# fusioninfer/fusioninfer

Hardware: NVIDIA H100
Metric: routing decisions/sec (4K-tok prompts x 1024 endpoints); achieved HBM GB/s (higher is better)
Workload: dtype u64

## Files before the change

fusioninfer_b200/csrc/engine.cu:

```cuda
#include <cuda_runtime.h>
#include <unistd.h>
#include <dlfcn.h>

#include <algorithm>
#include <atomic>
#include <chrono>
#include <cmath>
#include <condition_variable>
#include <cstdio>
#include <cstdlib>
#include <cstring>
#include <functional>
#include <memory>
#include <mutex>
#include <string>
#include <thread>
#include <unordered_set>
#include <vector>

#include <sched.h>

#include "../../include/fi_epp.h"
#include "cuda_owned.h"
#include "kernels.cuh"
// ... 149 lines not shown

  fi_epp_config cfg;
  std::mutex mu;
  std::string err;
  int sm_count = 132;
  uint32_t MP = 0;
  uint32_t W = 0;
  uint32_t P = 0;
  bool fast_hash = false;

  static constexpr int kMaxFeedSlices = 16;
  Event ev_copy[kMaxFeedSlices];
  uint32_t feed_slices = 8;
  DevPtr<uint64_t> d_chain2;
  DevPtr<uint32_t> d_nblocks2;
  Event ev_in, ev_a[2], ev_b[2];
  Event ev_pick;
  Event ev_plain;
  uint64_t pipe_seq = 0;
  static constexpr int kTicketRing = 8;
  Event ev_ticket[kTicketRing];
  uint64_t tickets = 0;
  uint64_t slot_ticket[2] = {~0ull, ~0ull};
  uint32_t slot_R[2] = {0, 0};
  Event ev_slot_read[2];
  Event ev_index, ev_user, ev_done, ev_ctr;

  DevPtr<uint8_t> d_prompts;
  DevPtr<uint64_t> d_offsets;
  DevPtr<uint64_t> d_h0;
  DevPtr<uint64_t> d_chain;
  DevPtr<uint32_t> d_nblocks;
  DevPtr<fi_pick> d_picks;
  Staging<fi_pick> ranked;
  Staging<uint32_t> subsets;
  Staging<uint16_t> counts;
  std::unique_ptr<ShardState> shard;
  PeerXchg px{};
  bool split_hash = false;
  uint32_t chain_rows = 0;
  DevPtr<unsigned long long> d_probed;
  DevPtr<uint32_t> d_work;
  PinnedPtr<fi_pick> h_picks;
  PinnedPtr<uint64_t> h_offsets;
  PinnedPtr<uint64_t> h_h0;
  PinnedPtr<uint32_t> h_nblocks;

// ... 819 lines not shown
    }
    LaunchScope ls(h, h->s_index.get(), K_INDEX);
    FI_CUDA(launch_index_clear_counted(h->ix.v, h->d_ctr.get(), h->dlru->clears.get(), r_total[k], h->dlru->ctr.get() + 2, lo, EL, h->rank, glog,
                                       h->s_index.get()));
  }
  return update_end(h, Readback::kIndexAndLru);
}

bool early_exit_hashing(const fi_epp* h, bool chains_wanted) {
  return h->world == 1 && h->fast_hash && !chains_wanted && h->cfg.lru_capacity == 0;
}

unsigned long long* hashed_counter(fi_epp* h) { return h->profiling ? h->d_probed.get() + 6 : nullptr; }

int run_hash(fi_epp* h, const uint8_t* d_prompts, const uint64_t* d_offsets, const uint64_t* d_h0, uint32_t r0,
             uint32_t R, cudaStream_t s, const IndexView* early) {
  uint64_t* chain = h->d_chain.get() + (size_t)r0 * h->MP;
  uint32_t* nb = h->d_nblocks.get() + r0;
  LaunchScope ls(h, s, K_HASH);
  if (h->fast_hash) {
    FI_CUDA(launch_hash_chain(d_prompts, d_offsets + r0, d_h0 + r0, R, h->cfg.block_bytes, h->cfg.max_blocks, h->MP,
                              chain, nb, h->sm_count, s, early, hashed_counter(h)));
  } else {
    FI_CUDA(launch_hash_generic(d_prompts, d_offsets + r0, d_h0 + r0, R, h->cfg.block_bytes, h->cfg.max_blocks, h->MP,
                                chain, nb, s));
  }
  return FI_OK;
}

int nccl_allgather_on(fi_epp* h, ncclComm_t comm, const void* send, void* recv, size_t bytes, cudaStream_t s) {
  int rc = g_nccl.AllGather(send, recv, bytes, ncclInt8, comm, s);
  if (rc != ncclSuccess)
    return fail(h, FI_ERR_COMM, std::string("ncclAllGather: ") + (g_nccl.GetErrorString ? g_nccl.GetErrorString(rc) : "error"));
  return FI_OK;
}
int nccl_allgather(fi_epp* h, const void* send, void* recv, size_t bytes) {
  return nccl_allgather_on(h, h->shard->comm, send, recv, bytes, h->s_main.get());
// ... 226 lines not shown
  const uint32_t S = h->feed_slices;
  if (feed && !sharded && h->fast_hash && S > 1 && R >= 64 * S && feed->offsets[R] >= (8ull << 20)) {
    uint8_t* dp = const_cast<uint8_t*>(c.prompts);
    const uint32_t per = (((R + S - 1) / S) + 31) & ~31u;
    uint32_t used = 0;
    for (uint32_t k = 0; k * per < R; ++k, ++used) {
      const uint32_t r0 = k * per, r1 = std::min(R, r0 + per);
      const uint64_t b0 = feed->offsets[r0], b1 = feed->offsets[r1];
      if (b1 > b0) FI_CUDA(cudaMemcpyAsync(dp + b0, feed->prompts + b0, b1 - b0, cudaMemcpyHostToDevice, h->s_copy.get()));
      FI_CUDA(cudaEventRecord(h->ev_copy[k].get(), h->s_copy.get()));
    }
    h->stats.h2d_bytes += feed->offsets[R];
    for (uint32_t k = 0; k < used; ++k) {
      const uint32_t r0 = k * per, Rk = std::min(per, R - r0);
      FI_CUDA(cudaStreamWaitEvent(h->s_main.get(), h->ev_copy[k].get(), 0));
      rc = run_hash(h, c.prompts, c.offsets, c.h0, r0, Rk, h->s_main.get(), early);
      if (rc != FI_OK) return rc;
      MatchParams ms = mp;
      ms.chain = mp.chain + (size_t)r0 * h->MP;
      ms.nblocks = mp.nblocks + r0;
      ms.offsets = mp.offsets ? mp.offsets + r0 : nullptr;
      ms.adapters = mp.adapters ? mp.adapters + r0 : nullptr;
      ms.subsets = mp.subsets ? mp.subsets + (size_t)r0 * mp.sub_pitch : nullptr;
      ms.h0 = mp.h0 + r0;
      ms.r_base = r0;
      ms.R = Rk;
      ms.out = mp.out ? mp.out + (size_t)r0 * h->P * std::max(c.k, 1u) : nullptr;
      ms.counts = mp.counts ? mp.counts + (size_t)r0 * h->cfg.endpoint_count : nullptr;
      ms.work_counter = h->d_work.get() + k;
      LaunchScope ls(h, h->s_main.get(), K_MATCH);
      FI_CUDA(launch_match_pick(ms, h->sm_count, h->s_main.get()));
    }
    return FI_OK;
  }
  if (feed && feed->offsets[R]) {
    FI_CUDA(cudaMemcpyAsync(const_cast<uint8_t*>(c.prompts), feed->prompts, feed->offsets[R], cudaMemcpyHostToDevice, h->s_main.get()));
    h->stats.h2d_bytes += feed->offsets[R];
  }
  if (!sharded) {
    rc = run_hash(h, c.prompts, c.offsets, c.h0, 0, R, h->s_main.get(), early);
    if (rc != FI_OK) return rc;
    LaunchScope ls(h, h->s_main.get(), K_MATCH);
    FI_CUDA(launch_match_pick(mp, h->sm_count, h->s_main.get()));
    return FI_OK;
  }

  if (h->split_hash && h->fast_hash && R >= 32 * h->world) {
    const uint32_t per = (((R + h->world - 1) / h->world) + 31) & ~31u;
    const uint32_t r0 = std::min(R, h->rank * per), r1 = std::min(R, r0 + per);
    if (r1 > r0) {
      rc = run_hash(h, c.prompts, c.offsets, c.h0, r0, r1 - r0, h->s_main.get(), nullptr);
      if (rc != FI_OK) return rc;
    }
    rc = nccl_allgather(h, h->d_chain.get() + (size_t)h->rank * per * h->MP, h->d_chain.get(), (size_t)per * h->MP * sizeof(uint64_t));
    if (rc != FI_OK) return rc;
// ... 60 lines not shown
  return FI_OK;
}

int issue_ticket(fi_epp* h, uint64_t* t) {
  FI_CUDA(cudaEventRecord(h->ev_ticket[h->tickets % fi_epp::kTicketRing].get(), h->s_main.get()));
  *t = h->tickets++;
  return FI_OK;
}

int submit_pick(fi_epp* h, const PickCall& c, cudaStream_t us, uint64_t* ticket, bool lagged) {
  const uint32_t R = c.R;
  int rc = settle_updates(h, lagged);
  if (rc != FI_OK) return rc;
  if (!h->d_chain2) {
    DevPtr<uint64_t> chain;
    DevPtr<uint32_t> nb;
    FI_CUDA(cuda_alloc(chain, (size_t)h->cfg.max_batch * h->MP));
    FI_CUDA(cuda_alloc(nb, h->cfg.max_batch));
    h->d_chain2 = std::move(chain);
    h->d_nblocks2 = std::move(nb);
  }
  if (!h->profiling && h->trace_call >= 0 && (long)h->stats.pick_calls >= h->trace_call &&
      (long)h->stats.pick_calls < h->trace_call + 3) {
    if ((long)h->stats.pick_calls == h->trace_call) {
      if (!h->ev_trace0) cuda_create(h->ev_trace0, cudaEventDefault);
      FI_CUDA(cudaStreamSynchronize(h->s_main.get()));
      FI_CUDA(cudaStreamSynchronize(h->s_a.get()));
      FI_CUDA(cudaEventRecord(h->ev_trace0.get(), h->s_main.get()));
      FI_CUDA(cudaStreamWaitEvent(h->s_a.get(), h->ev_trace0.get(), 0));
    }
    h->tracing = true;
  } else if (h->tracing && (long)h->stats.pick_calls >= h->trace_call + 3) {
    h->tracing = false;
  }
  const uint32_t slot = (uint32_t)(h->pipe_seq & 1);
  uint64_t* chain = slot ? h->d_chain2.get() : h->d_chain.get();
  uint32_t* nb = slot ? h->d_nblocks2.get() : h->d_nblocks.get();
  FI_CUDA(cudaEventRecord(h->ev_in.get(), us));
  FI_CUDA(cudaStreamWaitEvent(h->s_a.get(), h->ev_in.get(), 0));
  if (h->pipe_seq >= 2) FI_CUDA(cudaStreamWaitEvent(h->s_a.get(), h->ev_b[slot].get(), 0));
  FI_CUDA(cudaStreamWaitEvent(h->s_a.get(), h->ev_plain.get(), 0));
  rc = wait_slot_readers(h, slot, h->s_a.get());
  if (rc != FI_OK) return rc;
  MatchParams mp;
  rc = prepare_match(h, c, chain, nb, mp);
  if (rc != FI_OK) return rc;
  const bool early = early_exit_hashing(h, c.chains_out != nullptr);
  if (early) FI_CUDA(cudaStreamWaitEvent(h->s_a.get(), h->ev_index.get(), 0));
  {
    LaunchScope ls(h, h->s_a.get(), K_HASH);
    FI_CUDA(launch_hash_chain(c.prompts, c.offsets, c.h0, R, h->cfg.block_bytes, h->cfg.max_blocks, h->MP, chain, nb,
                              h->sm_count, h->s_a.get(), early ? &mp.ix : nullptr, hashed_counter(h)));
  }
  FI_CUDA(cudaEventRecord(h->ev_a[slot].get(), h->s_a.get()));
  FI_CUDA(cudaStreamWaitEvent(h->s_main.get(), h->ev_a[slot].get(), 0));
  mp.work_counter = h->d_work.get() + 8 + slot;
  {
    LaunchScope ls(h, h->s_main.get(), K_MATCH);
    FI_CUDA(launch_match_pick(mp, h->sm_count, h->s_main.get()));
  }
  rc = copy_chains_out(h, chain, c.chains_out, R, cudaMemcpyDeviceToDevice, h->s_main.get());
  if (rc != FI_OK) return rc;
  FI_CUDA(cudaEventRecord(h->ev_b[slot].get(), h->s_main.get()));
  FI_CUDA(cudaEventRecord(h->ev_pick.get(), h->s_main.get()));
  rc = issue_ticket(h, ticket);
  if (rc != FI_OK) return rc;
  h->slot_ticket[slot] = *ticket;
// ... 212 lines not shown
  if (const char* e = std::getenv("FI_EPP_FEED_SLICES")) {
    const long v = std::strtol(e, nullptr, 10);
    h->feed_slices = (uint32_t)std::min<long>(std::max<long>(v, 1), fi_epp::kMaxFeedSlices);
  }
  for (Event* e : {&h->ev_index, &h->ev_user, &h->ev_done, &h->ev_ctr}) FI_TRY(cuda_create(*e));
  FI_TRY(cudaEventRecord(h->ev_index.get(), h->s_index.get()));
  const uint64_t R = cfg->max_batch;
  h->chain_rows = (uint32_t)((R + 31) / 32 * 32);
  if (cfg->endpoint_count < cfg->num_endpoints) h->chain_rows += 32 * (FI_MAX_RANKS + 1);
  if (const char* e = std::getenv("FI_EPP_SHARD_HASH")) h->split_hash = std::strcmp(e, "split") == 0;
  FI_TRY(cuda_alloc(h->d_prompts, h->cfg.max_prompt_bytes + 64));
  FI_TRY(cuda_alloc(h->d_offsets, R + 1));
  FI_TRY(cuda_alloc(h->d_h0, R));
  FI_TRY(cuda_alloc(h->d_chain, (size_t)h->chain_rows * h->MP));
  FI_TRY(cuda_alloc(h->d_nblocks, h->chain_rows));
  FI_TRY(cuda_alloc(h->d_picks, R * h->P));
  FI_TRY(cuda_alloc(h->d_probed, 8));
  FI_TRY(cudaMemset(h->d_probed.get(), 0, 8 * sizeof(unsigned long long)));
  FI_TRY(cuda_alloc(h->d_work, 16));
  FI_TRY(cudaMemset(h->d_work.get(), 0, 16 * sizeof(uint32_t)));
  FI_TRY(cuda_alloc(h->h_picks, R * h->P));
  FI_TRY(cuda_alloc(h->h_offsets, R + 1));
  FI_TRY(cuda_alloc(h->h_h0, R));
  FI_TRY(cuda_alloc(h->h_nblocks, R));

  FI_TRY(cuda_alloc(h->d_ctr, 1));
  FI_TRY(cudaMemset(h->d_ctr.get(), 0, sizeof(IndexCounters)));
  FI_TRY(cuda_alloc(h->h_ctr, 1));
  std::memset(h->h_ctr.get(), 0, sizeof(IndexCounters));
  {
// ... 1341 lines not shown
```

fusioninfer_b200/csrc/hash_kernels.cu:

```cuda
#include "kernels.cuh"
#include "xxh64.cuh"
#include "xxh64_sm100.cuh"
#include "index_device.cuh"

namespace fi {

namespace {

__device__ __forceinline__ uint64_t make_evict_first_policy() {
  uint64_t pol;
  asm volatile("createpolicy.fractional.L2::evict_first.b64 %0, 1.0;\n" : "=l"(pol));
  return pol;
}
__device__ __forceinline__ uint4 ld_stream_v4(const uint4* p, uint64_t pol) {
  uint4 v;
  asm volatile("ld.global.nc.L1::evict_first.L2::cache_hint.v4.u32 {%0, %1, %2, %3}, [%4], %5;\n"
               : "=r"(v.x), "=r"(v.y), "=r"(v.z), "=r"(v.w)
               : "l"(p), "l"(pol));
  return v;
}

struct Stripe {
  uint32_t w[8];
};
// ... 55 lines not shown
  const uint32_t sh = (uint32_t)(addr & 7) * 8;
  XAcc2 a = xacc2_init();
  if constexpr (STRIPES == 0) {
#pragma unroll 2
    for (uint32_t s = 0; s < B / 32; ++s) xacc2_stripe_at(a, wp + 4 * (uint64_t)s, sh);
  } else {
#pragma unroll
    for (int s = 0; s < STRIPES; ++s) xacc2_stripe_at(a, wp + 4 * s, sh);
  }
  return xacc2_finish(a, (uint64_t)B + 8);
}

enum : int { kHashFull = 0, kHashFullCounted = 1, kHashEarly = 2 };

__device__ __forceinline__ uint32_t ld_volatile_shared(const uint32_t* p) { return *reinterpret_cast<const volatile uint32_t*>(p); }
__device__ __forceinline__ uint64_t ld_chain_cta(const uint64_t* p) {
  uint64_t v;
  asm volatile("ld.relaxed.cta.global.u64 %0, [%1];\n" : "=l"(v) : "l"(p) : "memory");
  return v;
}

template <int STRIPES, int WALK, int WARPS, int MODE>
__global__ void __launch_bounds__(WARPS * 32, 32 / WARPS) hash_chain_kernel(const uint8_t* __restrict__ prompts,
                                                                   const uint64_t* __restrict__ offsets,
                                                                   const uint64_t* __restrict__ h0, uint32_t R,
                                                                   uint32_t M, uint32_t MP,
                                                                   uint64_t* __restrict__ chain,
                                                                   uint32_t* __restrict__ nblocks,
                                                                   uint32_t block_bytes, const IndexView ix,
                                                                   unsigned long long* hashed) {
  constexpr bool EARLY = MODE == kHashEarly;
  const uint32_t B = STRIPES ? STRIPES * 32 : block_bytes;
  constexpr uint32_t BPL = STRIPES == 4 || STRIPES == 0 ? 1 : 2;
  constexpr uint32_t kFuseReq = 32 * WALK;
  constexpr uint32_t kFuseHashWarps = WARPS - WALK - (EARLY ? 1 : 0);
  constexpr uint32_t kFuseRing = WARPS * kFuseRingBytesPerWarp / (WALK * 4 * 32 * 16);
  constexpr uint32_t kJobs = kFuseReq / (4 * BPL);
  __shared__ __align__(16) ulonglong2 s_ring[kFuseRing][WALK][4][32];
  __shared__ uint64_t s_full[kFuseRing], s_empty[kFuseRing];
  __shared__ const uint8_t* s_base[kFuseReq];
  __shared__ uint32_t s_n[kFuseReq];
  __shared__ uint32_t s_groups;
  __shared__ uint32_t s_stop[EARLY ? kFuseReq : 1], s_walked[EARLY ? WALK : 1], s_hashed;

  const uint32_t tid = threadIdx.x, lane = tid & 31, warp = tid >> 5;
  const uint32_t r_tile = blockIdx.x * kFuseReq;
  if (tid == 0) {
    s_groups = 0;
    for (uint32_t s = 0; s < kFuseRing; ++s) {
      mbar_init(&s_full[s], kJobs * 32);
      mbar_init(&s_empty[s], WALK * 32);
    }
    if constexpr (EARLY)
      for (uint32_t w = 0; w < WALK; ++w) s_walked[w] = 0;
    if constexpr (MODE != kHashFull) s_hashed = 0;
  }
  __syncthreads();
  if (tid < kFuseReq) {
    const uint32_t r = r_tile + tid;
    uint32_t n = 0;
    const uint8_t* base = prompts;
    if (r < R) {
      const uint64_t off = offsets[r];
      const uint64_t nb64 = (offsets[r + 1] - off) / B;
      n = nb64 > M ? M : (uint32_t)nb64;
      base = prompts + off;
      nblocks[r] = n;
    }
    s_n[tid] = n;
    s_base[tid] = base;
    if constexpr (EARLY) s_stop[tid] = 0xFFFFFFFFu;
    if constexpr (MODE == kHashFullCounted)
      if (n) atomicAdd(&s_hashed, n);
    atomicMax(&s_groups, (n + 7) / 8);
  }
  __syncthreads();
  const uint32_t ng = s_groups;
  if constexpr (MODE == kHashFullCounted)
    if (tid == 0 && s_hashed) atomicAdd(hashed, (unsigned long long)s_hashed);

  if constexpr (EARLY) {
    if (warp == WALK) {
      uint32_t done_g[WALK];
      bool live[WALK];
#pragma unroll
      for (int j = 0; j < WALK; ++j) {
        done_g[j] = 0;
        live[j] = r_tile + j * 32 + lane < R && s_n[j * 32 + lane] > 0;
      }
#pragma unroll 1
      for (;;) {
        uint32_t gw[WALK];
        bool any = false, fresh = false;
#pragma unroll
        for (int j = 0; j < WALK; ++j) {
          gw[j] = ld_volatile_shared(&s_walked[j]);
          live[j] = live[j] && done_g[j] * 8 < s_n[j * 32 + lane];
          any = any || live[j];
          fresh = fresh || (live[j] && gw[j] > done_g[j]);
        }
        if (!__any_sync(0xFFFFFFFFu, any)) break;
        if (!__any_sync(0xFFFFFFFFu, fresh)) {
          __nanosleep(64);
          continue;
        }
        __threadfence_block();
        uint64_t hk[WALK];
#pragma unroll
        for (int j = 0; j < WALK; ++j) {
          const uint32_t q = j * 32 + lane;
          hk[j] = 0;
          if (live[j] && gw[j] > done_g[j]) {
            const uint32_t i = min(gw[j] * 8, s_n[q]) - 1;
            hk[j] = ld_chain_cta(chain + (uint64_t)(r_tile + q) * MP + i);
          }
        }
#pragma unroll
        for (int j = 0; j < WALK; ++j) {
          const uint32_t q = j * 32 + lane;
          if (live[j] && gw[j] > done_g[j]) {
            if (index_find(ix, hk[j]) == SLOT_MISS) {
              *reinterpret_cast<volatile uint32_t*>(&s_stop[q]) = gw[j];
              live[j] = false;
            }
            done_g[j] = gw[j];
          }
        }
      }
      return;
    }
  }

  if (warp >= WALK) {
    const uint64_t pol = make_evict_first_policy();
    const uint32_t b = lane & 7;
#pragma unroll 1
    for (uint32_t t = warp - WALK - (EARLY ? 1 : 0); t < ng * kJobs; t += kFuseHashWarps) {
      const uint32_t g = t / kJobs, job = t % kJobs;
      const uint32_t i = g * 8 + b;
      uint32_t q[BPL];
      bool ok[BPL], al[BPL], mis = false;
      const uint8_t* src[BPL];
      uint64_t pre[BPL];
#pragma unroll
      for (uint32_t k = 0; k < BPL; ++k) {
        q[k] = job * 4 * BPL + k * 4 + (lane >> 3);
        ok[k] = i < s_n[q[k]];
        if constexpr (EARLY) ok[k] = ok[k] && g < ld_volatile_shared(&s_stop[q[k]]);
        src[k] = s_base[q[k]] + (uint64_t)i * B;
        al[k] = (reinterpret_cast<uintptr_t>(src[k]) & 15) == 0;
        mis = mis || (ok[k] && !al[k]);
      }
// ... 35 lines not shown
      uint64_t* ring = reinterpret_cast<uint64_t*>(s_ring[slot]);
#pragma unroll
      for (uint32_t k = 0; k < BPL; ++k)
        if (ok[k]) ring[(((q[k] >> 5) * 4 + (b >> 1)) * 32 + (q[k] & 31)) * 2 + (b & 1)] = pre[k];
      mbar_arrive(&s_full[slot]);
    }
    return;
  }

  const uint32_t r = r_tile + warp * 32 + lane;
  const bool valid = r < R;
  const uint32_t n = s_n[warp * 32 + lane];
  uint64_t h = valid ? h0[r] : 0;
  const uint32_t MP2 = MP / 2;
  ulonglong2* out = reinterpret_cast<ulonglong2*>(chain) + (uint64_t)(valid ? r : 0) * MP2;
  uint32_t ng_full = valid ? n / 8 : 0;
#pragma unroll
  for (int d = 16; d > 0; d >>= 1) ng_full = min(ng_full, __shfl_xor_sync(0xFFFFFFFFu, ng_full, d));

  ulonglong2 in[4], res[4];
  auto take = [&](uint32_t g) {
    const uint32_t slot = g % kFuseRing;
    mbar_wait(&s_full[slot], (g / kFuseRing) & 1);
#pragma unroll
    for (int k = 0; k < 4; ++k) in[k] = lds16(&s_ring[slot][warp][k][lane]);
    mbar_arrive(&s_empty[slot]);
  };

  auto publish = [&](uint32_t g) {
    if constexpr (EARLY) {
      __syncwarp();
      if (lane == 0) {
        __threadfence_block();
        *reinterpret_cast<volatile uint32_t*>(&s_walked[warp]) = g + 1;
      }
    }
  };
  auto hashed_group = [&](uint32_t g) { return !EARLY || g < ld_volatile_shared(&s_stop[warp * 32 + lane]); };

  uint32_t g = 0;
#pragma unroll 1
  for (; g < ng_full; ++g) {
    take(g);
#pragma unroll
    for (int k = 0; k < 4; ++k) {
      h = chain_step(in[k].x, h);
      res[k].x = h;
      h = chain_step(in[k].y, h);
      res[k].y = h;
    }
    if constexpr (EARLY) {
      if (!hashed_group(g))
#pragma unroll
        for (int k = 0; k < 4; ++k) res[k] = make_ulonglong2(0, 0);
    }
    ulonglong2* o = out + g * 4;
#pragma unroll
    for (int k = 0; k < 4; ++k) st_row16(o + k, res[k]);
    publish(g);
  }
#pragma unroll 1
  for (; g < ng; ++g) {
    take(g);
    ulonglong2* o = out + g * 4;
    const uint32_t i0 = g * 8;
    const bool hg = hashed_group(g);
#pragma unroll
    for (int k = 0; k < 4; ++k) {
      ulonglong2 v;
      uint64_t t = chain_step(in[k].x, h);
      const bool v0 = i0 + 2 * k < n && hg;
      h = v0 ? t : h;
      v.x = v0 ? t : 0;
      t = chain_step(in[k].y, h);
      const bool v1 = i0 + 2 * k + 1 < n && hg;
      h = v1 ? t : h;
      v.y = v1 ? t : 0;
      if (valid) st_row16(o + k, v);
    }
    publish(g);
  }
  if (valid) {
    const ulonglong2 z = make_ulonglong2(0, 0);
    for (uint32_t u = g * 4; u < MP2; ++u) st_row16(out + u, z);
  }
  if constexpr (EARLY) {
    if (hashed && warp == 0 && lane == 0 && s_hashed) atomicAdd(hashed, (unsigned long long)s_hashed);
  }
}

__global__ void __launch_bounds__(128) hash_generic_kernel(const uint8_t* __restrict__ prompts,
                                                          const uint64_t* __restrict__ offsets,
                                                          const uint64_t* __restrict__ h0, uint32_t R, uint32_t B,
                                                          uint32_t M, uint32_t MP, uint64_t* __restrict__ chain,
                                                          uint32_t* __restrict__ nblocks) {
  const uint32_t r = blockIdx.x * 128 + threadIdx.x;
  if (r >= R) return;
  const uint64_t off = offsets[r];
  const uint64_t len = offsets[r + 1] - off;
  const uint64_t nb64 = len / B;
  const uint32_t n = nb64 > M ? M : (uint32_t)nb64;
  nblocks[r] = n;
// ... 4 lines not shown
    ChainMsg m{base + (uint64_t)i * B, B, h, true};
    h = xxh64_msg(m);
    out[i] = h;
  }
  for (uint32_t i = n; i < MP; ++i) out[i] = 0;
}

}

template <int STRIPES, int MODE>
static void launch_hash_chain_tile(uint32_t walk, uint32_t warps, uint32_t grid, cudaStream_t s, const uint8_t* prompts,
                                   const uint64_t* offsets, const uint64_t* h0, uint32_t R, uint32_t B, uint32_t M,
                                   uint32_t MP, uint64_t* chain, uint32_t* nblocks, const IndexView& ix,
                                   unsigned long long* hashed) {
  if (warps == 16)
    hash_chain_kernel<STRIPES, 2, 16, MODE><<<grid, 512, 0, s>>>(prompts, offsets, h0, R, M, MP, chain, nblocks, B, ix, hashed);
  else if (walk == 2)
    hash_chain_kernel<STRIPES, 2, 32, MODE><<<grid, 1024, 0, s>>>(prompts, offsets, h0, R, M, MP, chain, nblocks, B, ix, hashed);
  else
    hash_chain_kernel<STRIPES, 1, 32, MODE><<<grid, 1024, 0, s>>>(prompts, offsets, h0, R, M, MP, chain, nblocks, B, ix, hashed);
}

template <int STRIPES>
static void launch_hash_chain_mode(uint32_t walk, uint32_t warps, uint32_t grid, cudaStream_t s, const uint8_t* prompts,
                                   const uint64_t* offsets, const uint64_t* h0, uint32_t R, uint32_t B, uint32_t M,
                                   uint32_t MP, uint64_t* chain, uint32_t* nblocks, const IndexView* early,
                                   unsigned long long* hashed) {
  if (early && warps == 16)
    hash_chain_kernel<STRIPES, 2, 16, kHashEarly><<<grid, 512, 0, s>>>(prompts, offsets, h0, R, M, MP, chain, nblocks, B,
                                                                        *early, hashed);
  else if (hashed)
    launch_hash_chain_tile<STRIPES, kHashFullCounted>(walk, warps, grid, s, prompts, offsets, h0, R, B, M, MP, chain, nblocks,
                                                      IndexView{}, hashed);
  else
    launch_hash_chain_tile<STRIPES, kHashFull>(walk, warps, grid, s, prompts, offsets, h0, R, B, M, MP, chain, nblocks,
                                               IndexView{}, nullptr);
}

cudaError_t launch_hash_chain_shape(uint32_t walk, uint32_t warps, const uint8_t* prompts, const uint64_t* offsets,
                                    const uint64_t* h0, uint32_t R, uint32_t B, uint32_t M, uint32_t MP, uint64_t* chain,
                                    uint32_t* nblocks, cudaStream_t s, const IndexView* early, unsigned long long* hashed) {
  if (R == 0) return cudaSuccess;
  if (!((warps == 32 && (walk == 1 || walk == 2)) || (warps == 16 && walk == 2))) return cudaErrorInvalidValue;
  const uint32_t grid = (R + 32 * walk - 1) / (32 * walk);
  if (B == 64)
    launch_hash_chain_mode<2>(walk, warps, grid, s, prompts, offsets, h0, R, B, M, MP, chain, nblocks, early, hashed);
  else if (B == 32)
    launch_hash_chain_mode<1>(walk, warps, grid, s, prompts, offsets, h0, R, B, M, MP, chain, nblocks, early, hashed);
  else if (B == 128)
    launch_hash_chain_mode<4>(walk, warps, grid, s, prompts, offsets, h0, R, B, M, MP, chain, nblocks, early, hashed);
  else if (B % 32 == 0)
    launch_hash_chain_mode<0>(walk, warps, grid, s, prompts, offsets, h0, R, B, M, MP, chain, nblocks, early, hashed);
  else
    return cudaErrorInvalidValue;
  return cudaGetLastError();
}

cudaError_t launch_hash_chain(const uint8_t* prompts, const uint64_t* offsets, const uint64_t* h0, uint32_t R,
                              uint32_t B, uint32_t M, uint32_t MP, uint64_t* chain, uint32_t* nblocks, int sm_count,
                              cudaStream_t s, const IndexView* early, unsigned long long* hashed) {
  const uint32_t walk = (R + 31) / 32 > (uint32_t)sm_count ? 2 : 1;
  const uint32_t warps = (R + 63) / 64 > (uint32_t)sm_count ? 16 : 32;
  return launch_hash_chain_shape(walk, warps, prompts, offsets, h0, R, B, M, MP, chain, nblocks, s, early, hashed);
}

cudaError_t launch_hash_generic(const uint8_t* prompts, const uint64_t* offsets, const uint64_t* h0, uint32_t R,
                                uint32_t B, uint32_t M, uint32_t MP, uint64_t* chain, uint32_t* nblocks,
                                cudaStream_t s) {
  if (R == 0) return cudaSuccess;
  hash_generic_kernel<<<(R + 127) / 128, 128, 0, s>>>(prompts, offsets, h0, R, B, M, MP, chain, nblocks);
  return cudaGetLastError();
}


}
```

fusioninfer_b200/csrc/kernels.cuh:

```cuda
#pragma once
#include <cuda_runtime.h>
#include <stdint.h>

#include "../../include/fi_epp.h"

namespace fi {

constexpr uint32_t SLOT_MISS = 0xFFFFFFFFu;
constexpr uint64_t KEY_EMPTY = 0ull;
constexpr uint64_t KEY_TOMB = ~0ull;
constexpr int BUCKET_KEYS = 4;

struct IndexView {
  uint64_t* keys;
  uint32_t* node_of;
  uint64_t* klog;
  uint32_t* rows;
  uint32_t* cnt;
  uint32_t* rmask;
  uint64_t bmask;
  uint64_t C;
  uint32_t W;
  uint32_t logW;
};
// ... 94 lines not shown
  uint32_t r_base;
  const uint64_t* h0;
  uint32_t lpm;
  uint32_t apply_pd, pd_decode, pd_prefill;
  double pd_threshold;
  fi_pick* out;
  unsigned long long* probed_blocks;
  uint32_t* work_counter;
  uint32_t lane_zero;
  uint32_t k;
  PeerXchg px;
  const uint32_t* subsets;
  uint32_t sub_pitch;
  const EndpointDev* eps;
  uint16_t* counts;
};

struct MergeParams {
  const fi_pick* gathered;
  uint32_t ranks, R, P;
  const uint32_t* nblocks;
  const uint64_t* offsets;
  const uint64_t* chain;
  const uint64_t* h0;
  uint32_t MP, E_global;
  uint32_t apply_pd, pd_decode, pd_prefill;
  double pd_threshold;
  fi_pick* out;
  PeerXchg px;
};

cudaError_t launch_hash_chain(const uint8_t* prompts, const uint64_t* offsets, const uint64_t* h0, uint32_t R,
                              uint32_t B, uint32_t M, uint32_t MP, uint64_t* chain, uint32_t* nblocks,
                              int sm_count, cudaStream_t s, const IndexView* early = nullptr,
                              unsigned long long* hashed = nullptr);
cudaError_t launch_hash_chain_shape(uint32_t walk, uint32_t warps, const uint8_t* prompts, const uint64_t* offsets,
                                    const uint64_t* h0, uint32_t R, uint32_t B, uint32_t M, uint32_t MP, uint64_t* chain,
                                    uint32_t* nblocks, cudaStream_t s, const IndexView* early = nullptr,
                                    unsigned long long* hashed = nullptr);
cudaError_t launch_hash_generic(const uint8_t* prompts, const uint64_t* offsets, const uint64_t* h0,
                                uint32_t R, uint32_t B, uint32_t M, uint32_t MP, uint64_t* chain,
                                uint32_t* nblocks, cudaStream_t s);

cudaError_t launch_index_set(IndexView ix, IndexCounters* ctr, const fi_index_op* ops, uint64_t n,
                             uint32_t ep_begin, uint32_t ep_count, uint32_t rank, GossipLog log, cudaStream_t s);
cudaError_t launch_index_clear(IndexView ix, IndexCounters* ctr, const fi_index_op* ops, uint64_t n,
                               uint32_t ep_begin, uint32_t ep_count, uint32_t rank, GossipLog log, cudaStream_t s);
cudaError_t launch_index_clear_counted(IndexView ix, IndexCounters* ctr, const fi_index_op* ops, uint64_t cap,
                                       const unsigned long long* n_dev, uint32_t ep_begin, uint32_t ep_count, uint32_t rank,
                                       GossipLog log, cudaStream_t s);
cudaError_t launch_index_remote_appear(IndexView ix, IndexCounters* ctr, const uint64_t* hashes, uint64_t n,
                                       uint32_t rank, cudaStream_t s);
cudaError_t launch_index_remote_vanish(IndexView ix, IndexCounters* ctr, const uint64_t* hashes, uint64_t n,
                                       uint32_t rank, cudaStream_t s);
// ... 36 lines not shown
```

fusioninfer_b200/csrc/match_kernels.cu:

```cuda
#include <climits>
#include <map>
#include <mutex>
#include <utility>

#include "bitslice.cuh"
#include "index_device.cuh"
#include "kernels.cuh"
#include "tiebreak.cuh"

namespace fi {

namespace {

constexpr int kWarps = 8;
#ifndef FI_MATCH_MIN_BLOCKS
#define FI_MATCH_MIN_BLOCKS 2
#endif
constexpr unsigned FULL = 0xFFFFFFFFu;

struct Best {
  double score;
  uint32_t e;
  uint32_t m;
  uint32_t k;
// ... 325 lines not shown
  const int lane = threadIdx.x & 31;
  const int t = lane % LPR;
  const int g = lane / LPR;
  uint64_t* const s_chain_base = s_mem + (size_t)(2 * warp) * p.MP;
  uint32_t* s_node = reinterpret_cast<uint32_t*>(s_mem + (size_t)2 * kWarps * p.MP) + (size_t)warp * p.MP;
  uint16_t* s_row = nullptr;
  if constexpr (COUNTS)
    s_row = reinterpret_cast<uint16_t*>(s_mem + (size_t)2 * kWarps * p.MP) + (size_t)2 * kWarps * p.MP +
            (size_t)warp * (p.st.Epad + 16);
  const IndexView ix = p.ix;
  const uint32_t P = COUNTS ? 0u : p.st.n_profiles;
  const char* row_base = reinterpret_cast<const char*>(ix.rows + t * VEC);
  const uint32_t row_bytes = 4u << ix.logW;
  const uint32_t zero_slot = (uint32_t)(ix.C + 2);

  const uint32_t row_units = p.MP / 2;
  auto stage = [&](uint32_t rr, uint64_t* dst) {
    const uint64_t* crow = p.chain + (uint64_t)rr * p.MP;
    for (uint32_t u = lane; u < row_units; u += 32) cp_async16(dst + 2 * u, crow + 2 * u);
  };
  uint32_t r_next = 0;
  if (lane == 0) r_next = take_ticket(p.work_counter, threadIdx.x & p.lane_zero);
  r_next = __shfl_sync(FULL, r_next, 0);
  int buf = 0;
  if (r_next < p.R) stage(r_next, s_chain_base);
  bool pf_ok = false;
  uint64_t pf_h = 0, pf_key = 0;
  uint32_t pf_node = 0;
  for (;;) {
    const uint32_t r = r_next;
    if (r >= p.R) break;
    if (lane == 0) r_next = take_ticket(p.work_counter, threadIdx.x & p.lane_zero);
    const uint32_t n = p.nblocks[r];
    uint32_t sub[VEC];
#pragma unroll
    for (int x = 0; x < VEC; ++x) {
      sub[x] = 0u;
      if constexpr (SUBSET) {
        const uint32_t wi = t * VEC + x;
        if (wi < p.sub_pitch) sub[x] = __ldg(p.subsets + (uint64_t)r * p.sub_pitch + wi);
      }
    }
    uint64_t* s_chain = s_chain_base + (size_t)buf * p.MP;
#ifdef FI_MATCH_TIMING
    const long long tm0 = clock64();
#endif
// ... 13 lines not shown
    }

#ifdef FI_MATCH_TIMING
    const long long tm1 = clock64();
#endif
    BitCounter cnt[VEC];
    uint32_t alive[VEC];
#pragma unroll
    for (int x = 0; x < VEC; ++x) {
      bc_clear(cnt[x]);
      alive[x] = 0xFFFFFFFFu;
    }
    uint32_t matched_rows = 0;
    bool real_miss = false;

    const uint32_t m_rows = resolve_request_nodes(ix, s_chain, s_node, n, lane, have_first, first_node);
    real_miss = m_rows < n;
    __syncwarp();
    r_next = __shfl_sync(FULL, r_next, 0);
    pf_ok = false;
    if (r_next < p.R) {
      stage(r_next, s_chain_base + (size_t)(buf ^ 1) * p.MP);
      pf_h = __ldg(p.chain + (uint64_t)r_next * p.MP);
    }
#ifdef FI_MATCH_TIMING
    const long long tm2 = clock64();
#endif
#pragma unroll 1
    for (uint32_t b0 = 0; b0 < m_rows; b0 += BATCH * G) {
      uint32_t w[VEC][BATCH];
#pragma unroll
      for (int qi = 0; qi < BATCH; ++qi) {
        const uint32_t j = b0 + qi * G + g;
        const uint32_t sn = j < m_rows ? s_node[j] : zero_slot;
        uint32_t tmp[VEC];
        load_row_words<VEC>(reinterpret_cast<const uint32_t*>(row_base + (uint64_t)sn * row_bytes), true, tmp);
#pragma unroll
// ... 25 lines not shown
      for (int x = 0; x < VEC; ++x) {
        uint32_t any = 0;
#pragma unroll
        for (int qi = 0; qi < BATCH; ++qi) any |= w[x][qi];
        if (__any_sync(FULL, any != 0)) bc_add<BATCH>(cnt[x], w[x]);
      }
      matched_rows = min(m_rows, b0 + BATCH * G);
      if (LPM) {
        bool any = false;
#pragma unroll
        for (int x = 0; x < VEC; ++x) any |= alive[x] != 0;
        if (!__ballot_sync(FULL, any)) break;
      }
    }

    if (r_next < p.R && !key_is_special(pf_h)) {
      pf_ok = true;
      if (lane < BUCKET_KEYS) {
        const uint64_t slot0 = (pf_h & ix.bmask) * BUCKET_KEYS + lane;
        pf_key = __ldg(ix.keys + slot0);
        pf_node = __ldg(ix.node_of + slot0);
      }
    }
#ifdef FI_MATCH_TIMING
    const long long tm3 = clock64();
#endif
    const bool nothing = matched_rows == 0;
    if (G > 1 && !nothing) {
#pragma unroll
      for (int x = 0; x < VEC; ++x) {
// ... 418 lines not shown
```

Baseline: 113.1 million.

## Inline early-exit index probing into hash walkers and trim match staging to valid entries

Removes the dedicated early-exit probe warp and its shared-memory publish/poll handshake. Each hash walker warp now prefetches the index bucket for its running hash and checks it on the next group, stopping stores once a miss is seen. The kernel records per-request valid chain lengths (nvalid), which the match kernel uses to stage only the valid part of each chain row. The chain-row prefetch is also moved after the row scan instead of overlapping it. This adds a nvalid buffer and plumbing, and the later staging may expose more copy latency.

```diff
diff --git a/fusioninfer_b200/csrc/engine.cu b/fusioninfer_b200/csrc/engine.cu
--- a/fusioninfer_b200/csrc/engine.cu
+++ b/fusioninfer_b200/csrc/engine.cu
@@ -187,6 +187,7 @@
   uint32_t feed_slices = 8;
   DevPtr<uint64_t> d_chain2;
   DevPtr<uint32_t> d_nblocks2;
+  DevPtr<uint32_t> d_nvalid2;
   Event ev_in, ev_a[2], ev_b[2];
   Event ev_pick;
   Event ev_plain;
@@ -204,6 +205,7 @@
   DevPtr<uint64_t> d_h0;
   DevPtr<uint64_t> d_chain;
   DevPtr<uint32_t> d_nblocks;
+  DevPtr<uint32_t> d_nvalid;
   DevPtr<fi_pick> d_picks;
   Staging<fi_pick> ranked;
   Staging<uint32_t> subsets;
@@ -1053,13 +1055,15 @@
 unsigned long long* hashed_counter(fi_epp* h) { return h->profiling ? h->d_probed.get() + 6 : nullptr; }
 
 int run_hash(fi_epp* h, const uint8_t* d_prompts, const uint64_t* d_offsets, const uint64_t* d_h0, uint32_t r0,
-             uint32_t R, cudaStream_t s, const IndexView* early) {
+             uint32_t R, cudaStream_t s, const IndexView* early, const uint32_t** nvalid = nullptr) {
   uint64_t* chain = h->d_chain.get() + (size_t)r0 * h->MP;
   uint32_t* nb = h->d_nblocks.get() + r0;
+  uint32_t* nv = h->d_nvalid.get() + r0;
+  if (nvalid) *nvalid = early && h->fast_hash && hash_chain_stops_early(R, h->sm_count) ? nv : nullptr;
   LaunchScope ls(h, s, K_HASH);
   if (h->fast_hash) {
     FI_CUDA(launch_hash_chain(d_prompts, d_offsets + r0, d_h0 + r0, R, h->cfg.block_bytes, h->cfg.max_blocks, h->MP,
-                              chain, nb, h->sm_count, s, early, hashed_counter(h)));
+                              chain, nb, h->sm_count, s, early, nv, hashed_counter(h)));
   } else {
     FI_CUDA(launch_hash_generic(d_prompts, d_offsets + r0, d_h0 + r0, R, h->cfg.block_bytes, h->cfg.max_blocks, h->MP,
                                 chain, nb, s));
@@ -1316,9 +1320,9 @@
     for (uint32_t k = 0; k < used; ++k) {
       const uint32_t r0 = k * per, Rk = std::min(per, R - r0);
       FI_CUDA(cudaStreamWaitEvent(h->s_main.get(), h->ev_copy[k].get(), 0));
-      rc = run_hash(h, c.prompts, c.offsets, c.h0, r0, Rk, h->s_main.get(), early);
+      MatchParams ms = mp;
+      rc = run_hash(h, c.prompts, c.offsets, c.h0, r0, Rk, h->s_main.get(), early, &ms.nvalid);
       if (rc != FI_OK) return rc;
-      MatchParams ms = mp;
       ms.chain = mp.chain + (size_t)r0 * h->MP;
       ms.nblocks = mp.nblocks + r0;
       ms.offsets = mp.offsets ? mp.offsets + r0 : nullptr;
@@ -1340,7 +1344,7 @@
     h->stats.h2d_bytes += feed->offsets[R];
   }
   if (!sharded) {
-    rc = run_hash(h, c.prompts, c.offsets, c.h0, 0, R, h->s_main.get(), early);
+    rc = run_hash(h, c.prompts, c.offsets, c.h0, 0, R, h->s_main.get(), early, &mp.nvalid);
     if (rc != FI_OK) return rc;
     LaunchScope ls(h, h->s_main.get(), K_MATCH);
     FI_CUDA(launch_match_pick(mp, h->sm_count, h->s_main.get()));
@@ -1431,11 +1435,13 @@
   if (rc != FI_OK) return rc;
   if (!h->d_chain2) {
     DevPtr<uint64_t> chain;
-    DevPtr<uint32_t> nb;
+    DevPtr<uint32_t> nb, nv;
     FI_CUDA(cuda_alloc(chain, (size_t)h->cfg.max_batch * h->MP));
     FI_CUDA(cuda_alloc(nb, h->cfg.max_batch));
+    FI_CUDA(cuda_alloc(nv, h->cfg.max_batch));
     h->d_chain2 = std::move(chain);
     h->d_nblocks2 = std::move(nb);
+    h->d_nvalid2 = std::move(nv);
   }
   if (!h->profiling && h->trace_call >= 0 && (long)h->stats.pick_calls >= h->trace_call &&
       (long)h->stats.pick_calls < h->trace_call + 3) {
@@ -1453,6 +1459,7 @@
   const uint32_t slot = (uint32_t)(h->pipe_seq & 1);
   uint64_t* chain = slot ? h->d_chain2.get() : h->d_chain.get();
   uint32_t* nb = slot ? h->d_nblocks2.get() : h->d_nblocks.get();
+  uint32_t* nv = slot ? h->d_nvalid2.get() : h->d_nvalid.get();
   FI_CUDA(cudaEventRecord(h->ev_in.get(), us));
   FI_CUDA(cudaStreamWaitEvent(h->s_a.get(), h->ev_in.get(), 0));
   if (h->pipe_seq >= 2) FI_CUDA(cudaStreamWaitEvent(h->s_a.get(), h->ev_b[slot].get(), 0));
@@ -1464,10 +1471,11 @@
   if (rc != FI_OK) return rc;
   const bool early = early_exit_hashing(h, c.chains_out != nullptr);
   if (early) FI_CUDA(cudaStreamWaitEvent(h->s_a.get(), h->ev_index.get(), 0));
+  if (early && hash_chain_stops_early(R, h->sm_count)) mp.nvalid = nv;
   {
     LaunchScope ls(h, h->s_a.get(), K_HASH);
     FI_CUDA(launch_hash_chain(c.prompts, c.offsets, c.h0, R, h->cfg.block_bytes, h->cfg.max_blocks, h->MP, chain, nb,
-                              h->sm_count, h->s_a.get(), early ? &mp.ix : nullptr, hashed_counter(h)));
+                              h->sm_count, h->s_a.get(), early ? &mp.ix : nullptr, nv, hashed_counter(h)));
   }
   FI_CUDA(cudaEventRecord(h->ev_a[slot].get(), h->s_a.get()));
   FI_CUDA(cudaStreamWaitEvent(h->s_main.get(), h->ev_a[slot].get(), 0));
@@ -1710,6 +1718,7 @@
   FI_TRY(cuda_alloc(h->d_h0, R));
   FI_TRY(cuda_alloc(h->d_chain, (size_t)h->chain_rows * h->MP));
   FI_TRY(cuda_alloc(h->d_nblocks, h->chain_rows));
+  FI_TRY(cuda_alloc(h->d_nvalid, h->chain_rows));
   FI_TRY(cuda_alloc(h->d_picks, R * h->P));
   FI_TRY(cuda_alloc(h->d_probed, 8));
   FI_TRY(cudaMemset(h->d_probed.get(), 0, 8 * sizeof(unsigned long long)));
diff --git a/fusioninfer_b200/csrc/hash_kernels.cu b/fusioninfer_b200/csrc/hash_kernels.cu
--- a/fusioninfer_b200/csrc/hash_kernels.cu
+++ b/fusioninfer_b200/csrc/hash_kernels.cu
@@ -93,11 +93,6 @@
 enum : int { kHashFull = 0, kHashFullCounted = 1, kHashEarly = 2 };
 
 __device__ __forceinline__ uint32_t ld_volatile_shared(const uint32_t* p) { return *reinterpret_cast<const volatile uint32_t*>(p); }
-__device__ __forceinline__ uint64_t ld_chain_cta(const uint64_t* p) {
-  uint64_t v;
-  asm volatile("ld.relaxed.cta.global.u64 %0, [%1];\n" : "=l"(v) : "l"(p) : "memory");
-  return v;
-}
 
 template <int STRIPES, int WALK, int WARPS, int MODE>
 __global__ void __launch_bounds__(WARPS * 32, 32 / WARPS) hash_chain_kernel(const uint8_t* __restrict__ prompts,
@@ -107,12 +102,13 @@
                                                                    uint64_t* __restrict__ chain,
                                                                    uint32_t* __restrict__ nblocks,
                                                                    uint32_t block_bytes, const IndexView ix,
-                                                                   unsigned long long* hashed) {
+                                                                   unsigned long long* hashed,
+                                                                   uint32_t* __restrict__ nvalid) {
   constexpr bool EARLY = MODE == kHashEarly;
   const uint32_t B = STRIPES ? STRIPES * 32 : block_bytes;
   constexpr uint32_t BPL = STRIPES == 4 || STRIPES == 0 ? 1 : 2;
   constexpr uint32_t kFuseReq = 32 * WALK;
-  constexpr uint32_t kFuseHashWarps = WARPS - WALK - (EARLY ? 1 : 0);
+  constexpr uint32_t kFuseHashWarps = WARPS - WALK;
   constexpr uint32_t kFuseRing = WARPS * kFuseRingBytesPerWarp / (WALK * 4 * 32 * 16);
   constexpr uint32_t kJobs = kFuseReq / (4 * BPL);
   __shared__ __align__(16) ulonglong2 s_ring[kFuseRing][WALK][4][32];
@@ -120,7 +116,7 @@
   __shared__ const uint8_t* s_base[kFuseReq];
   __shared__ uint32_t s_n[kFuseReq];
   __shared__ uint32_t s_groups;
-  __shared__ uint32_t s_stop[EARLY ? kFuseReq : 1], s_walked[EARLY ? WALK : 1], s_hashed;
+  __shared__ uint32_t s_stop[EARLY ? kFuseReq : 1], s_hashed;
 
   const uint32_t tid = threadIdx.x, lane = tid & 31, warp = tid >> 5;
   const uint32_t r_tile = blockIdx.x * kFuseReq;
@@ -130,8 +126,6 @@
       mbar_init(&s_full[s], kJobs * 32);
       mbar_init(&s_empty[s], WALK * 32);
     }
-    if constexpr (EARLY)
-      for (uint32_t w = 0; w < WALK; ++w) s_walked[w] = 0;
     if constexpr (MODE != kHashFull) s_hashed = 0;
   }
   __syncthreads();
@@ -158,63 +152,11 @@
   if constexpr (MODE == kHashFullCounted)
     if (tid == 0 && s_hashed) atomicAdd(hashed, (unsigned long long)s_hashed);
 
-  if constexpr (EARLY) {
-    if (warp == WALK) {
-      uint32_t done_g[WALK];
-      bool live[WALK];
-#pragma unroll
-      for (int j = 0; j < WALK; ++j) {
-        done_g[j] = 0;
-        live[j] = r_tile + j * 32 + lane < R && s_n[j * 32 + lane] > 0;
-      }
-#pragma unroll 1
-      for (;;) {
-        uint32_t gw[WALK];
-        bool any = false, fresh = false;
-#pragma unroll
-        for (int j = 0; j < WALK; ++j) {
-          gw[j] = ld_volatile_shared(&s_walked[j]);
-          live[j] = live[j] && done_g[j] * 8 < s_n[j * 32 + lane];
-          any = any || live[j];
-          fresh = fresh || (live[j] && gw[j] > done_g[j]);
-        }
-        if (!__any_sync(0xFFFFFFFFu, any)) break;
-        if (!__any_sync(0xFFFFFFFFu, fresh)) {
-          __nanosleep(64);
-          continue;
-        }
-        __threadfence_block();
-        uint64_t hk[WALK];
-#pragma unroll
-        for (int j = 0; j < WALK; ++j) {
-          const uint32_t q = j * 32 + lane;
-          hk[j] = 0;
-          if (live[j] && gw[j] > done_g[j]) {
-            const uint32_t i = min(gw[j] * 8, s_n[q]) - 1;
-            hk[j] = ld_chain_cta(chain + (uint64_t)(r_tile + q) * MP + i);
-          }
-        }
-#pragma unroll
-        for (int j = 0; j < WALK; ++j) {
-          const uint32_t q = j * 32 + lane;
-          if (live[j] && gw[j] > done_g[j]) {
-            if (index_find(ix, hk[j]) == SLOT_MISS) {
-              *reinterpret_cast<volatile uint32_t*>(&s_stop[q]) = gw[j];
-              live[j] = false;
-            }
-            done_g[j] = gw[j];
-          }
-        }
-      }
-      return;
-    }
-  }
-
   if (warp >= WALK) {
     const uint64_t pol = make_evict_first_policy();
     const uint32_t b = lane & 7;
 #pragma unroll 1
-    for (uint32_t t = warp - WALK - (EARLY ? 1 : 0); t < ng * kJobs; t += kFuseHashWarps) {
+    for (uint32_t t = warp - WALK; t < ng * kJobs; t += kFuseHashWarps) {
       const uint32_t g = t / kJobs, job = t % kJobs;
       const uint32_t i = g * 8 + b;
       uint32_t q[BPL];
@@ -280,10 +222,6 @@
   uint64_t h = valid ? h0[r] : 0;
   const uint32_t MP2 = MP / 2;
   ulonglong2* out = reinterpret_cast<ulonglong2*>(chain) + (uint64_t)(valid ? r : 0) * MP2;
-  uint32_t ng_full = valid ? n / 8 : 0;
-#pragma unroll
-  for (int d = 16; d > 0; d >>= 1) ng_full = min(ng_full, __shfl_xor_sync(0xFFFFFFFFu, ng_full, d));
-
   ulonglong2 in[4], res[4];
   auto take = [&](uint32_t g) {
     const uint32_t slot = g % kFuseRing;
@@ -293,17 +231,49 @@
     mbar_arrive(&s_empty[slot]);
   };
 
-  auto publish = [&](uint32_t g) {
-    if constexpr (EARLY) {
-      __syncwarp();
-      if (lane == 0) {
-        __threadfence_block();
-        *reinterpret_cast<volatile uint32_t*>(&s_walked[warp]) = g + 1;
-      }
-    }
-  };
-  auto hashed_group = [&](uint32_t g) { return !EARLY || g < ld_volatile_shared(&s_stop[warp * 32 + lane]); };
-
+  if constexpr (EARLY) {
+    const uint32_t q = warp * 32 + lane;
+    uint32_t stop = 0xFFFFFFFFu;
+    bool probing = false;
+    BucketRegs bk;
+#pragma unroll 1
+    for (uint32_t g = 0; g < ng; ++g) {
+      take(g);
+      if (probing && bucket_scan(bk, h) == BUCKET_KEYS) {
+        stop = g;
+        *reinterpret_cast<volatile uint32_t*>(&s_stop[q]) = g;
+      }
+      probing = false;
+      const uint32_t i0 = g * 8;
+#pragma unroll
+      for (int k = 0; k < 4; ++k) {
+        uint64_t t = chain_step(in[k].x, h);
+        const bool v0 = i0 + 2 * k < n;
+        h = v0 ? t : h;
+        res[k].x = v0 ? t : 0;
+        t = chain_step(in[k].y, h);
+        const bool v1 = i0 + 2 * k + 1 < n;
+        h = v1 ? t : h;
+        res[k].y = v1 ? t : 0;
+      }
+      if (valid && i0 < n && g < stop) {
+        ulonglong2* o = out + g * 4;
+#pragma unroll
+        for (int k = 0; k < 4; ++k) st_row16(o + k, res[k]);
+        if (i0 + 8 < n && !key_is_special(h)) {
+          bk = bucket_load_keys(ix, h & ix.bmask);
+          probing = true;
+        }
+      }
+    }
+    if (valid) nvalid[r] = stop == 0xFFFFFFFFu ? n : min(n, 8 * stop);
+    if (hashed && warp == 0 && lane == 0 && s_hashed) atomicAdd(hashed, (unsigned long long)s_hashed);
+    return;
+  }
+
+  uint32_t ng_full = valid ? n / 8 : 0;
+#pragma unroll
+  for (int d = 16; d > 0; d >>= 1) ng_full = min(ng_full, __shfl_xor_sync(0xFFFFFFFFu, ng_full, d));
   uint32_t g = 0;
 #pragma unroll 1
   for (; g < ng_full; ++g) {
@@ -315,43 +285,32 @@
       h = chain_step(in[k].y, h);
       res[k].y = h;
     }
-    if constexpr (EARLY) {
-      if (!hashed_group(g))
-#pragma unroll
-        for (int k = 0; k < 4; ++k) res[k] = make_ulonglong2(0, 0);
-    }
     ulonglong2* o = out + g * 4;
 #pragma unroll
     for (int k = 0; k < 4; ++k) st_row16(o + k, res[k]);
-    publish(g);
   }
 #pragma unroll 1
   for (; g < ng; ++g) {
     take(g);
     ulonglong2* o = out + g * 4;
     const uint32_t i0 = g * 8;
-    const bool hg = hashed_group(g);
 #pragma unroll
     for (int k = 0; k < 4; ++k) {
       ulonglong2 v;
       uint64_t t = chain_step(in[k].x, h);
-      const bool v0 = i0 + 2 * k < n && hg;
+      const bool v0 = i0 + 2 * k < n;
       h = v0 ? t : h;
       v.x = v0 ? t : 0;
       t = chain_step(in[k].y, h);
-      const bool v1 = i0 + 2 * k + 1 < n && hg;
+      const bool v1 = i0 + 2 * k + 1 < n;
       h = v1 ? t : h;
       v.y = v1 ? t : 0;
       if (valid) st_row16(o + k, v);
     }
-    publish(g);
   }
   if (valid) {
     const ulonglong2 z = make_ulonglong2(0, 0);
     for (uint32_t u = g * 4; u < MP2; ++u) st_row16(out + u, z);
-  }
-  if constexpr (EARLY) {
-    if (hashed && warp == 0 && lane == 0 && s_hashed) atomicAdd(hashed, (unsigned long long)s_hashed);
   }
 }
 
@@ -386,21 +345,24 @@
                                    uint32_t MP, uint64_t* chain, uint32_t* nblocks, const IndexView& ix,
                                    unsigned long long* hashed) {
   if (warps == 16)
-    hash_chain_kernel<STRIPES, 2, 16, MODE><<<grid, 512, 0, s>>>(prompts, offsets, h0, R, M, MP, chain, nblocks, B, ix, hashed);
+    hash_chain_kernel<STRIPES, 2, 16, MODE><<<grid, 512, 0, s>>>(prompts, offsets, h0, R, M, MP, chain, nblocks, B, ix, hashed,
+                                                                 nullptr);
   else if (walk == 2)
-    hash_chain_kernel<STRIPES, 2, 32, MODE><<<grid, 1024, 0, s>>>(prompts, offsets, h0, R, M, MP, chain, nblocks, B, ix, hashed);
+    hash_chain_kernel<STRIPES, 2, 32, MODE><<<grid, 1024, 0, s>>>(prompts, offsets, h0, R, M, MP, chain, nblocks, B, ix, hashed,
+                                                                  nullptr);
   else
-    hash_chain_kernel<STRIPES, 1, 32, MODE><<<grid, 1024, 0, s>>>(prompts, offsets, h0, R, M, MP, chain, nblocks, B, ix, hashed);
+    hash_chain_kernel<STRIPES, 1, 32, MODE><<<grid, 1024, 0, s>>>(prompts, offsets, h0, R, M, MP, chain, nblocks, B, ix, hashed,
+                                                                  nullptr);
 }
 
 template <int STRIPES>
 static void launch_hash_chain_mode(uint32_t walk, uint32_t warps, uint32_t grid, cudaStream_t s, const uint8_t* prompts,
                                    const uint64_t* offsets, const uint64_t* h0, uint32_t R, uint32_t B, uint32_t M,
                                    uint32_t MP, uint64_t* chain, uint32_t* nblocks, const IndexView* early,
-                                   unsigned long long* hashed) {
+                                   uint32_t* nvalid, unsigned long long* hashed) {
   if (early && warps == 16)
     hash_chain_kernel<STRIPES, 2, 16, kHashEarly><<<grid, 512, 0, s>>>(prompts, offsets, h0, R, M, MP, chain, nblocks, B,
-                                                                        *early, hashed);
+                                                                        *early, hashed, nvalid);
   else if (hashed)
     launch_hash_chain_tile<STRIPES, kHashFullCounted>(walk, warps, grid, s, prompts, offsets, h0, R, B, M, MP, chain, nblocks,
                                                       IndexView{}, hashed);
@@ -411,29 +373,33 @@
 
 cudaError_t launch_hash_chain_shape(uint32_t walk, uint32_t warps, const uint8_t* prompts, const uint64_t* offsets,
                                     const uint64_t* h0, uint32_t R, uint32_t B, uint32_t M, uint32_t MP, uint64_t* chain,
-                                    uint32_t* nblocks, cudaStream_t s, const IndexView* early, unsigned long long* hashed) {
+                                    uint32_t* nblocks, cudaStream_t s, const IndexView* early, uint32_t* nvalid,
+                                    unsigned long long* hashed) {
   if (R == 0) return cudaSuccess;
+  if (early && !nvalid) return cudaErrorInvalidValue;
   if (!((warps == 32 && (walk == 1 || walk == 2)) || (warps == 16 && walk == 2))) return cudaErrorInvalidValue;
   const uint32_t grid = (R + 32 * walk - 1) / (32 * walk);
   if (B == 64)
-    launch_hash_chain_mode<2>(walk, warps, grid, s, prompts, offsets, h0, R, B, M, MP, chain, nblocks, early, hashed);
+    launch_hash_chain_mode<2>(walk, warps, grid, s, prompts, offsets, h0, R, B, M, MP, chain, nblocks, early, nvalid, hashed);
   else if (B == 32)
-    launch_hash_chain_mode<1>(walk, warps, grid, s, prompts, offsets, h0, R, B, M, MP, chain, nblocks, early, hashed);
+    launch_hash_chain_mode<1>(walk, warps, grid, s, prompts, offsets, h0, R, B, M, MP, chain, nblocks, early, nvalid, hashed);
   else if (B == 128)
-    launch_hash_chain_mode<4>(walk, warps, grid, s, prompts, offsets, h0, R, B, M, MP, chain, nblocks, early, hashed);
+    launch_hash_chain_mode<4>(walk, warps, grid, s, prompts, offsets, h0, R, B, M, MP, chain, nblocks, early, nvalid, hashed);
   else if (B % 32 == 0)
-    launch_hash_chain_mode<0>(walk, warps, grid, s, prompts, offsets, h0, R, B, M, MP, chain, nblocks, early, hashed);
+    launch_hash_chain_mode<0>(walk, warps, grid, s, prompts, offsets, h0, R, B, M, MP, chain, nblocks, early, nvalid, hashed);
   else
     return cudaErrorInvalidValue;
   return cudaGetLastError();
 }
 
+bool hash_chain_stops_early(uint32_t R, int sm_count) { return (R + 63) / 64 > (uint32_t)sm_count; }
+
 cudaError_t launch_hash_chain(const uint8_t* prompts, const uint64_t* offsets, const uint64_t* h0, uint32_t R,
                               uint32_t B, uint32_t M, uint32_t MP, uint64_t* chain, uint32_t* nblocks, int sm_count,
-                              cudaStream_t s, const IndexView* early, unsigned long long* hashed) {
+                              cudaStream_t s, const IndexView* early, uint32_t* nvalid, unsigned long long* hashed) {
   const uint32_t walk = (R + 31) / 32 > (uint32_t)sm_count ? 2 : 1;
-  const uint32_t warps = (R + 63) / 64 > (uint32_t)sm_count ? 16 : 32;
-  return launch_hash_chain_shape(walk, warps, prompts, offsets, h0, R, B, M, MP, chain, nblocks, s, early, hashed);
+  const uint32_t warps = hash_chain_stops_early(R, sm_count) ? 16 : 32;
+  return launch_hash_chain_shape(walk, warps, prompts, offsets, h0, R, B, M, MP, chain, nblocks, s, early, nvalid, hashed);
 }
 
 cudaError_t launch_hash_generic(const uint8_t* prompts, const uint64_t* offsets, const uint64_t* h0, uint32_t R,
diff --git a/fusioninfer_b200/csrc/kernels.cuh b/fusioninfer_b200/csrc/kernels.cuh
--- a/fusioninfer_b200/csrc/kernels.cuh
+++ b/fusioninfer_b200/csrc/kernels.cuh
@@ -132,6 +132,7 @@
   uint32_t sub_pitch;
   const EndpointDev* eps;
   uint16_t* counts;
+  const uint32_t* nvalid;
 };
 
 struct MergeParams {
@@ -151,11 +152,12 @@
 cudaError_t launch_hash_chain(const uint8_t* prompts, const uint64_t* offsets, const uint64_t* h0, uint32_t R,
                               uint32_t B, uint32_t M, uint32_t MP, uint64_t* chain, uint32_t* nblocks,
                               int sm_count, cudaStream_t s, const IndexView* early = nullptr,
-                              unsigned long long* hashed = nullptr);
+                              uint32_t* nvalid = nullptr, unsigned long long* hashed = nullptr);
+bool hash_chain_stops_early(uint32_t R, int sm_count);
 cudaError_t launch_hash_chain_shape(uint32_t walk, uint32_t warps, const uint8_t* prompts, const uint64_t* offsets,
                                     const uint64_t* h0, uint32_t R, uint32_t B, uint32_t M, uint32_t MP, uint64_t* chain,
                                     uint32_t* nblocks, cudaStream_t s, const IndexView* early = nullptr,
-                                    unsigned long long* hashed = nullptr);
+                                    uint32_t* nvalid = nullptr, unsigned long long* hashed = nullptr);
 cudaError_t launch_hash_generic(const uint8_t* prompts, const uint64_t* offsets, const uint64_t* h0,
                                 uint32_t R, uint32_t B, uint32_t M, uint32_t MP, uint64_t* chain,
                                 uint32_t* nblocks, cudaStream_t s);
diff --git a/fusioninfer_b200/csrc/match_kernels.cu b/fusioninfer_b200/csrc/match_kernels.cu
--- a/fusioninfer_b200/csrc/match_kernels.cu
+++ b/fusioninfer_b200/csrc/match_kernels.cu
@@ -363,22 +363,27 @@
   const uint32_t row_bytes = 4u << ix.logW;
   const uint32_t zero_slot = (uint32_t)(ix.C + 2);
 
-  const uint32_t row_units = p.MP / 2;
-  auto stage = [&](uint32_t rr, uint64_t* dst) {
+  auto stage = [&](uint32_t rr, uint64_t* dst, uint32_t nv) {
     const uint64_t* crow = p.chain + (uint64_t)rr * p.MP;
-    for (uint32_t u = lane; u < row_units; u += 32) cp_async16(dst + 2 * u, crow + 2 * u);
+    for (uint32_t u = lane; u < (nv + 1) / 2; u += 32) cp_async16(dst + 2 * u, crow + 2 * u);
   };
+  auto valid_entries = [&](uint32_t rr) { return p.nvalid ? min(p.nvalid[rr], p.nblocks[rr]) : p.nblocks[rr]; };
   uint32_t r_next = 0;
   if (lane == 0) r_next = take_ticket(p.work_counter, threadIdx.x & p.lane_zero);
   r_next = __shfl_sync(FULL, r_next, 0);
   int buf = 0;
-  if (r_next < p.R) stage(r_next, s_chain_base);
+  uint32_t nv_next = 0;
+  if (r_next < p.R) {
+    nv_next = valid_entries(r_next);
+    stage(r_next, s_chain_base, nv_next);
+  }
   bool pf_ok = false;
   uint64_t pf_h = 0, pf_key = 0;
   uint32_t pf_node = 0;
   for (;;) {
     const uint32_t r = r_next;
     if (r >= p.R) break;
+    const uint32_t nv = nv_next;
     if (lane == 0) r_next = take_ticket(p.work_counter, threadIdx.x & p.lane_zero);
     const uint32_t n = p.nblocks[r];
     uint32_t sub[VEC];
@@ -422,13 +427,13 @@
     uint32_t matched_rows = 0;
     bool real_miss = false;
 
-    const uint32_t m_rows = resolve_request_nodes(ix, s_chain, s_node, n, lane, have_first, first_node);
+    const uint32_t m_rows = resolve_request_nodes(ix, s_chain, s_node, nv, lane, have_first, first_node);
     real_miss = m_rows < n;
     __syncwarp();
     r_next = __shfl_sync(FULL, r_next, 0);
     pf_ok = false;
     if (r_next < p.R) {
-      stage(r_next, s_chain_base + (size_t)(buf ^ 1) * p.MP);
+      nv_next = valid_entries(r_next);
       pf_h = __ldg(p.chain + (uint64_t)r_next * p.MP);
     }
 #ifdef FI_MATCH_TIMING
@@ -484,6 +489,7 @@
       }
     }
 
+    if (r_next < p.R) stage(r_next, s_chain_base + (size_t)(buf ^ 1) * p.MP, nv_next);
     if (r_next < p.R && !key_is_special(pf_h)) {
       pf_ok = true;
       if (lane < BUCKET_KEYS) {
```

Result: faster. 114.9 million, median of 6 (+1.6%).
